# phhusson/SpeechSeparation

Measured on AMD Instinct MI355X. Metric: separated row-frames/sec, batch64 8s@16kHz, higher is better.
Workload: dtype f32 io/accumulate, fp16x2-split operands (22-bit operands, 3 f16 MFMA terms; a2*b2 term dropped)

## Files before the change

speechseparation_amd/csrc/api.hip:

```cpp
#include "api_internal.h"
#include "metrics_host.h"
#include "sections_host.h"

#include <cmath>
#include <cstdarg>
#include <cstdio>

namespace bsrnn::host {

std::atomic<long long> g_dbg[5];

static thread_local char g_err[512] = "";
int fail(int code, const char* fmt, ...)
{
    va_list ap;
    va_start(ap, fmt);
    vsnprintf(g_err, sizeof(g_err), fmt, ap);
    va_end(ap);
    return code;
}

hipError_t UploadRing::reserve(size_t bytes)
{
    if (bytes <= cap) return hipSuccess;
// ... 169 lines not shown
                (void)hipFree(t.d[0]);
                return fail(BSRNN_EHIP, "task table: %s", hipGetErrorString(e));
            }
        }
        c->chain_tasks.emplace(Ms[i], t);
    }
    return 0;
}
int ensure_tasks(bsrnn_ctx* c, int M) { return ensure_tasks(c, &M, 1); }

void gemm_slot(bsrnn_ctx* c, bool gemv, int slot, const float* X, int ldx, float* Y, int ldy, const float* R, int ldr,
               const float* Mul, int ldm, float* tap, int M, int epi, hipStream_t s)
{
    GemmLaunch g;
    memset(&g, 0, sizeof g);
    g.range_flag = c->d_range;
    g.jobs = c->d_jobs + c->slots.job0[slot];
    g.tiles = c->d_tiles + c->slots.tile0[slot];
    g.n_tiles = c->slots.ntiles[slot];
    g.tile_n = c->slots.tile_n[slot];
    g.X = X; g.ldx = ldx; g.Y = Y; g.ldy = ldy; g.R = R; g.ldr = ldr; g.Mul = Mul; g.ldm = ldm;
    g.tap = tap; g.ldt = c->LDP; g.M = M; g.epilogue = epi;
    if (gemv && M <= 2 * GEMV_MAX_FRAME_ROWS) launch_gemv(g, s);
    else launch_gemm(g, s);
}

static const PlanKnobs& plan_knobs()
{
    static const PlanKnobs knobs = [] {
        auto is = [](const char* name, const char* value) { const char* e = getenv(name); return e && !strcmp(e, value); };
        const char *tk = getenv("BSRNN_TIME_KERNEL"), *s8 = getenv("BSRNN_TIME_SEQ8");
        if (tk && *tk && strcmp(tk, "fused") && strcmp(tk, "v3")) fprintf(stderr, "bsrnn: unknown BSRNN_TIME_KERNEL='%s' (v3 | fused), using fused\n", tk);
        return PlanKnobs{!is("BSRNN_BAND_PAIR", "0"), !is("BSRNN_BAND_FC", "gemm"), !is("BSRNN_TIME_KERNEL", "v3"), s8 ? atoi(s8) : -1,
                         gemm_mode(), lstm_mode(), device_cus()};
    }();
    return knobs;
}
Flow plan_call(const bsrnn_ctx* c, int C, int T, bool gemv, bool overlap)
{
    return plan_call(c->K, C, T, gemv, overlap, plan_knobs(), PlanState{force_f32(), c->fused, c->band_pair_off, c->overlap_env, c->overlap_off});
}

struct Part {
    int C, T;
    Flow f;
    hipStream_t s;
    const float* Xf; float* Yf; float* tap;
    float *A1, *A2, *P, *Z0, *Z1, *HB0, *HB1, *H1;
    int* band_flags;
    const float* state_in; float* state_out;
    size_t state_slab;
    const float* wave; float* wave_out; int64_t n;
    const int64_t* lens;
    int64_t wave_stride, out_stride;
    const int2* tasks[2]; int n_tasks[2];
    const bsrnn_ctx::OvlTable* ovl;
    int ovl_base;
    hipEvent_t band_done[2];
    const int* row_frames;
};

Part make_part(bsrnn_ctx* c, int row0, int C, int T, hipStream_t s, int j = 0)
{
    Part p;
    memset(&p, 0, sizeof p);
    const size_t m0 = (size_t)row0 * T, KH = (size_t)c->K * HID;
    p.C = C; p.T = T; p.s = s;
// ... 37 lines not shown
    case MS_BANDSPLIT: {
        StageScope sc(c, ST_BANDSPLIT, s);
        if (f.chains) {
            ChainLaunch g;
            if (!chain_launch(c, p, CHAIN_SPLIT, g)) break;
            g.Xin = p.Xf; g.ldx = c->LDP; g.Z = p.Z0; g.ldz = KH;
            launch_mlp_chain(g, CHAIN_SPLIT, s);
            break;
        }
        gemm_slot(c, f.gemv, PRE0, p.Xf, c->LDP, p.A1, c->LDA, nullptr, 0, nullptr, 0, nullptr, M, EPI_LEAKY, s);
        gemm_slot(c, f.gemv, PRE2, p.A1, c->LDA, p.P, c->LDP, nullptr, 0, nullptr, 0, nullptr, M, EPI_LEAKY, s);
        gemm_slot(c, f.gemv, FC0, p.P, c->LDP, p.A1, c->LDA, nullptr, 0, nullptr, 0, nullptr, M, EPI_LEAKY, s);
        gemm_slot(c, f.gemv, FC2, p.A1, c->LDA, p.A2, c->LDA, nullptr, 0, nullptr, 0, nullptr, M, EPI_LEAKY, s);
        gemm_slot(c, f.gemv, FC4, p.A2, c->LDA, p.Z0, KH, nullptr, 0, nullptr, 0, nullptr, M, EPI_LINEAR, s);
        break;
    }
    case MS_BAND0: case MS_BAND1: {
        const int blk = stage == MS_BAND1;
        StageScope sc(c, ST_BAND_LSTM, s);
        if (f.band == BAND_SMALL) {
            launch_band_block_small(p.Z0, p.Z1, c->bandW16[blk][0], c->bandB[blk][0], c->bandW16[blk][1], c->bandB[blk][1],
                                    c->bandFc16[blk], c->bandFcB[blk], M, K, c->d_range, s);
            break;
        }
        const bool parts = f.band == BAND_PAIR_PARTS;
        const float* zi = parts && blk ? p.Z1 : p.Z0;
        if (f.band != BAND_LAYERS) {
            OvlConsumer oc = {nullptr, 0, 0, nullptr, 0, 2};
            const bool cons = p.ovl && blk;
            if (cons)
                oc = OvlConsumer{c->d_ovl + OVL_HEAD, p.T, c->overlap_sabotage ? 200000 : OVL_SPIN_LIMIT, p.ovl->band_order, p.ovl_base, f.seqs == 8 ? 3 : 2};
            launch_band_pair(zi, p.HB0, p.HB1, c->bandW16[blk][0], c->bandB[blk][0], c->bandW16[blk][1], c->bandB[blk][1], M, K, c->d_range, s,
                             parts ? c->bandFc16[blk] : nullptr, parts ? c->bandFcB[blk] : nullptr, p.band_flags, cons ? &oc : nullptr, nullptr, 0,
                             p.ovl ? p.band_done[blk] : nullptr);
            break;
        }
        launch_band_lstm(zi, p.HB0, c->bandW[blk][0], c->bandW16[blk][0], c->bandB[blk][0], M, K, 64, c->d_range, s, f.lstm_f32);
        launch_band_lstm(p.HB0, p.HB1, c->bandW[blk][1], c->bandW16[blk][1], c->bandB[blk][1], M, K, 128, c->d_range, s, f.lstm_f32);
        break;
    }
    case MS_BANDFC0: case MS_BANDFC1: {
        const int blk = stage == MS_BANDFC1;
        if (f.band == BAND_SMALL || f.band == BAND_PAIR_PARTS) break;
        StageScope sc(c, ST_BAND_FC, s);
        gemm_slot(c, f.gemv, BLK_FC0 + 2 * blk, p.HB1, 2 * HID, p.Z1, HID, p.Z0, HID, nullptr, 0, nullptr, M * K, EPI_RES, s);
        break;
    }
    case MS_TIME0: case MS_TIME1: {
        const int blk = stage == MS_TIME1;
        StageScope sc(c, ST_TIME_LSTM, s);
        const bool first_of_parts = f.band == BAND_PAIR_PARTS && !blk;
        OvlProducer op = {nullptr, nullptr, 0};
        if (p.ovl) op = OvlProducer{c->d_ovl + blk * c->ovl_stride, c->overlap_sabotage ? nullptr : c->d_ovl + blk * c->ovl_stride + OVL_HEAD, p.ovl_base};
        launch_time_lstm(first_of_parts ? p.Z0 : p.Z1, first_of_parts ? p.Z1 : (f.time_fc ? p.Z0 : p.H1), c->timeW[blk], c->timeW16[blk], c->timeB[blk],
                         p.state_in ? p.state_in + blk * p.state_slab : nullptr, p.state_out ? p.state_out + blk * p.state_slab : nullptr,
                         p.C, p.T, K, c->d_range, s, f.lstm_f32, f.seqs, f.time_fc ? c->timeFc16[blk] : nullptr, f.time_fc ? c->timeFcB[blk] : nullptr,
                         f.band == BAND_PAIR_PARTS ? p.HB1 : nullptr, p.ovl ? &op : nullptr, p.row_frames);
        break;
    }
    case MS_TIMEFC0: case MS_TIMEFC1: {
        const int blk = stage == MS_TIMEFC1;
        if (f.time_fc) break;
        StageScope sc(c, ST_TIME_FC, s);
        gemm_slot(c, f.gemv, BLK_FC1 + 2 * blk, p.H1, HID, p.Z0, HID, p.Z1, HID, nullptr, 0, nullptr, M * K, EPI_RES, s);
        break;
    }
    case MS_MASK: {
// ... 1754 lines not shown
```

speechseparation_amd/csrc/kernels.h:

```cpp
#pragma once
#include <hip/hip_runtime.h>
#include <stdint.h>

#include "descriptors.h"
#include "stream_rows_host.h"
#include "resample_bank_host.h"
#include "train_ragged_host.h"
#include "pool_host.h"
#include "convolve_host.h"
#include "convolve_stream_host.h"
#include "metrics_host.h"
#include "remix_host.h"
#include "critic_host.h"

namespace bsrnn {

enum GemmEpilogue {
    EPI_LINEAR = 0,
    EPI_LEAKY = 1,
    EPI_RES = 2,
    EPI_MASK = 3
};

struct GemmLaunch {
// ... 36 lines not shown
void launch_mlp_chain(const ChainLaunch& g, int chain, hipStream_t stream);

struct OvlProducer { int* resident; int* prog; int base; };
struct OvlConsumer { const int* prog; int T; int spin_limit; const int* order; int base; int wg_shift; };
constexpr int OVL_SPIN_LIMIT = 20000000;
void launch_ovl_gate(const int* resident, int target, int* range_flag, int spin_limit, hipStream_t stream);
int device_cus();
#if defined(__HIPCC__)
__device__ __forceinline__ bool ovl_wait_rows(const int* prog, int m_first, int m_last, int T, int K, int k_first, int k_last, int limit, int base, int wg_shift)
{
    typedef const int __attribute__((address_space(1)))* gci;
    const gci pg = (gci)prog;
    const int r_a = m_first / T, r_b = m_last / T;
    const unsigned long long t0 = __builtin_amdgcn_s_memrealtime();
    for (int r = r_a; r <= r_b; ++r) {
        const int t_last = r < r_b ? T - 1 : m_last - r * T;
        const int need = base + (t_last >> 2) + 1;
        for (int wg = (r * K + k_first) >> wg_shift; wg <= (r * K + k_last) >> wg_shift; ++wg)
            while (__hip_atomic_load(pg + wg, __ATOMIC_RELAXED, __HIP_MEMORY_SCOPE_AGENT) < need) {
                __builtin_amdgcn_s_sleep(16);
                if (__builtin_amdgcn_s_memrealtime() - t0 > (unsigned long long)limit) return false;
            }
    }
    __builtin_amdgcn_fence(__ATOMIC_ACQUIRE, "agent");
    asm volatile("s_waitcnt vmcnt(0)" ::: "memory");
    return true;
}
#endif

void launch_band_lstm(const float* xin, float* hout, const float* wpk, const void* wpk16, const float* bias,
                      int N, int L, int IN, int* range_flag, hipStream_t stream, bool f32);
void launch_band_pair(const float* z, float* hb0, float* hb1, const void* w0pk16, const float* bias0, const void* w1pk16, const float* bias1,
                      int N, int L, int* range_flag, hipStream_t stream, const void* fc16, const float* fcb, int* flags,
                      const OvlConsumer* ovl = nullptr, int* zero_words = nullptr, int zero_n = 0, hipEvent_t done = nullptr);
void launch_band_block_small(const float* zin, float* zout, const void* w0pk16, const float* bias0, const void* w1pk16, const float* bias1,
                             const void* fc16, const float* fcb, int N, int L, int* range_flag, hipStream_t stream);
int lstm_mode();
void launch_time_lstm(const float* zin, float* hout, const float* wpk, const void* wpk16, const float* bias,
                      const float* state_in, float* state_out, int R, int T, int K, int* range_flag, hipStream_t stream,
                      bool f32, int seqs, const void* fc16 = nullptr, const float* fcb = nullptr, const float* part = nullptr,
                      const OvlProducer* ovl = nullptr,
                      const int* row_frames = nullptr);

constexpr int LSTM_TRAIN_CHUNKS = 64;
constexpr int LSTM_TRAIN_MAX_CHUNKS = 256;
constexpr int GEMM_GROUP = 12;
struct TrainGemmJob {
    const float* A; const float* B; float* C; const float* bias;
    int lda, ldb, ldc;
    int M, N, K;
    int tiles_x, tiles_y, rpc;
};
struct TrainGemmGroup { TrainGemmJob j[GEMM_GROUP]; int first[GEMM_GROUP + 1]; int count; };
struct ReduceJob { const float* part; float* out1; float* out2; int n1, n2, chunks; };
struct ReduceGroup { ReduceJob j[GEMM_GROUP]; int first[GEMM_GROUP + 1]; int count; };
void launch_sgemm_group(TrainGemmGroup& g, int trans_b, int accumulate, int leaky, hipStream_t stream);
size_t tn_group_scratch_floats(const TrainGemmGroup& g);
void launch_sgemm_tn_group(const TrainGemmGroup& g, float* scratch, int L, int shift, hipStream_t stream);
size_t sgemm_tn_scratch_floats(int M, int N1, int N2);
void train_reduction_layout(int M, int N1, int N2, int out[2]);
size_t colsum_scratch_floats(int M, int cols);
void launch_sgemm(const float* A, int lda, const float* B, int ldb, int trans_b, float* C, int ldc, int M, int N, int K,
                  int accumulate, const float* bias, int leaky, hipStream_t stream);
void launch_sgemm_tn(const float* A, int lda, const float* B, int ldb, float* out, float* colsum, float* scratch, int M, int N1, int N2,
                     int L, int shift, hipStream_t stream);
void launch_colsum(const float* A, int lda, float* out, float* scratch, int M, int cols, hipStream_t stream);
void launch_adamw(float* p, const float* g, float* m, float* v, size_t n, float lr, double b1, double b2, float eps, float wd,
// ... 142 lines not shown
```

speechseparation_amd/csrc/lstm.hip:

```cpp
#include "kernels.h"
#include <hip/hip_ext.h>

#include <cstdio>
#include <cstdlib>
#include <cstring>
#include <type_traits>

namespace bsrnn {

typedef float v4f __attribute__((ext_vector_type(4)));

constexpr int BAND_NLDS = 2;
constexpr int BAND_NLDS64 = 0;

__device__ __forceinline__ float fast_sigmoid(float x)
{
    return __builtin_amdgcn_rcpf(1.0f + __expf(-x));
}
__device__ __forceinline__ float fast_tanh(float x)
{
    return 2.0f * __builtin_amdgcn_rcpf(1.0f + __expf(-2.0f * x)) - 1.0f;
}
__device__ __forceinline__ v4f exp2_4(const v4f x)
{
    return (v4f){__builtin_amdgcn_exp2f(x[0]), __builtin_amdgcn_exp2f(x[1]), __builtin_amdgcn_exp2f(x[2]), __builtin_amdgcn_exp2f(x[3])};
}
__device__ __forceinline__ v4f rcp4(const v4f x)
{
    return (v4f){__builtin_amdgcn_rcpf(x[0]), __builtin_amdgcn_rcpf(x[1]), __builtin_amdgcn_rcpf(x[2]), __builtin_amdgcn_rcpf(x[3])};
}

constexpr int BAND_OCC = 2;
template <int IN>
// ... 92 lines not shown
            c[r] = fg * c[r] + ig * gg;
            hbuf[nxt][(4 * q + r) * SH + 16 * wave + l15] = og * fast_tanh(c[r]);
        }
        if (more) xstore(nxt, xn);
        __syncthreads();
        if (n0 + o_row < N)
            *reinterpret_cast<float4*>(hout + ((size_t)(n0 + o_row) * L + t) * (2 * HID) + dir * HID + 4 * o_c4) =
                *reinterpret_cast<const float4*>(&hbuf[nxt][o_row * SH + 4 * o_c4]);
    }
}

typedef _Float16 h8v __attribute__((ext_vector_type(8)));
typedef _Float16 h4v __attribute__((ext_vector_type(4)));
typedef unsigned u4v __attribute__((ext_vector_type(4)));

__device__ __forceinline__ void split_h2(float v, _Float16& p0, _Float16& p1)
{
    asm("" : "+v"(v));
    p0 = (_Float16)v;
    p1 = (_Float16)__builtin_fmaf(-(float)p0, 2048.f, v * 2048.f);
}

template <int IN, bool PART>
struct BandLds {
    static constexpr int NLDS = IN == 128 ? BAND_NLDS : BAND_NLDS64;
    static constexpr int XPL = 0;
    static constexpr int HPL = XPL + 2 * 2 * IN * 16 * 2;
    static constexpr int W2 = HPL + 2 * 2 * HID * 16 * 2;
    static constexpr int BIAS = W2 + (NLDS ? 4 * NLDS * 4 * 64 : 1) * 16;
    static constexpr int FC = BIAS + (4 * HID + HID) * 4;
    static constexpr int BYTES = FC + (PART ? 4 * 2 * 2 * 64 : 1) * 16;
};

template <int IN, bool TRACE, bool PART>
__device__ __forceinline__ void band_layer_body(char* const lds, const int dir, const int tile,
                                                const float* __restrict__ xin, float* __restrict__ hout,
                                                const uint4* __restrict__ wpk, const float* __restrict__ bias,
                                                int N, int L, int* __restrict__ range_flag, unsigned long long* __restrict__ dbg,
                                                const uint4* __restrict__ wfc, const float* __restrict__ bfc)
{
    static_assert(!PART || IN == 2 * HID, "the fc share is formed by the second layer");
    unsigned long long tp[5] = {0, 0, 0, 0, 0}, tq = 0;
    auto stamp = [&](int k) { if (TRACE) { const unsigned long long now = __builtin_amdgcn_s_memrealtime(); tp[k] += now - tq; tq = now; } };
    if (TRACE) tq = __builtin_amdgcn_s_memrealtime();
    constexpr int NBX = IN / 32, NBH = HID / 32, NB = NBX + NBH;
    constexpr bool PLANES_IN = IN == 2 * HID;
    constexpr bool PLANES_OUT = IN == HID;
    constexpr int NLDS = IN == 128 ? BAND_NLDS : BAND_NLDS64;
    constexpr int XV = IN / 64;
    using LD = BandLds<IN, PART>;
    auto& xpl = *reinterpret_cast<_Float16 (*)[2][2][IN * 16]>(lds + LD::XPL);
    auto& hpl = *reinterpret_cast<_Float16 (*)[2][2][HID * 16]>(lds + LD::HPL);
    uint4* const w2lds = reinterpret_cast<uint4*>(lds + LD::W2);
    float* const bias_lds = reinterpret_cast<float*>(lds + LD::BIAS);
    uint4* const fclds = reinterpret_cast<uint4*>(lds + LD::FC);
    const int n0 = tile * 16;
    const int tid = threadIdx.x, lane = tid & 63, wave = tid >> 6;
    const int l15 = lane & 15, q = lane >> 4;

    h8v w[NB][4][2];
    {
        const uint4* wp = wpk + ((size_t)(dir * 4 + wave) * NB * 4 * 2) * 64 + lane;
#pragma unroll
        for (int b = 0; b < NB; ++b)
#pragma unroll
            for (int gte = 0; gte < 4; ++gte)
#pragma unroll
                for (int pc = 0; pc < 2; ++pc) {
                    const uint4 v = wp[((b * 4 + gte) * 2 + pc) * 64];
                    if (pc == 1 && b >= NB - NLDS)
                        w2lds[((wave * NLDS + (b - (NB - NLDS))) * 4 + gte) * 64 + lane] = v;
                    else
                        w[b][gte][pc] = __builtin_bit_cast(h8v, v);
                }
    }
    bias_lds[tid] = bias[dir * 256 + tid];
    if (PART) {
#pragma unroll
        for (int i = 0; i < 4; ++i) fclds[(wave * 4 + i) * 64 + lane] = wfc[((size_t)(wave * 4 + 2 * dir) * 2 + i) * 64 + lane];
    }
#pragma unroll
    for (int b = 0; b < NB; ++b)
#pragma unroll
        for (int gte = 0; gte < 4; ++gte) {
            asm volatile("" : "+v"(w[b][gte][0]));
            if (b < NB - NLDS) asm volatile("" : "+v"(w[b][gte][1]));
        }
    v4f cv = {0.f, 0.f, 0.f, 0.f};

    int xrow[XV], xcol[XV];
#pragma unroll
    for (int i = 0; i < XV; ++i) {
        const int u = tid + 256 * i;
        xrow[i] = u / (IN / 4);
        xcol[i] = u % (IN / 4);
    }
    auto xload = [&](int t, u4v* dst) {
#pragma unroll
        for (int i = 0; i < XV; ++i) {
            int row = n0 + xrow[i];
            row = row < N ? row : N - 1;
            dst[i] = *reinterpret_cast<const u4v*>(xin + ((size_t)row * L + t) * IN + 4 * xcol[i]);
        }
    };
    float amax = 0.f;
    auto xstore = [&](int slot, const u4v* src) {
#pragma unroll
        for (int i = 0; i < XV; ++i) {
            if (PLANES_IN) {
                const int piece = xcol[i] >> 4, k8 = xcol[i] & 15;
                *reinterpret_cast<u4v*>(&xpl[slot][piece][(k8 * 16 + xrow[i]) * 8]) = src[i];
            } else {
                const v4f v = __builtin_bit_cast(v4f, src[i]);
                h4v p0, p1;
#pragma unroll
                for (int e = 0; e < 4; ++e) {
                    amax = __builtin_fmaxf(amax, __builtin_fabsf(v[e]));
                    _Float16 a, b2;
                    split_h2(v[e], a, b2);
                    p0[e] = a; p1[e] = b2;
// ... 10 lines not shown
    const v4f zero4 = {0.f, 0.f, 0.f, 0.f};
    const int frag = (q * 16 + l15) * 8;
    const float* const bias_l = &bias_lds[16 * wave + 4 * q];
    auto block_mfma = [&](const int b, const h8v a0, const h8v a1) {
        h8v w2[4];
#pragma unroll
        for (int gte = 0; gte < 4; ++gte)
            w2[gte] = b >= NB - NLDS ? __builtin_bit_cast(h8v, w2lds[((wave * NLDS + (b - (NB - NLDS))) * 4 + gte) * 64 + lane]) : w[b][gte][1];
#pragma unroll
        for (int gte = 0; gte < 4; ++gte)
            hi[gte] = __builtin_amdgcn_mfma_f32_16x16x32_f16(w[b][gte][0], a0, b == 0 ? *reinterpret_cast<const v4f*>(bias_l + gte * HID) : hi[gte], 0, 0, 0);
#pragma unroll
        for (int gte = 0; gte < 4; ++gte) lo[gte] = __builtin_amdgcn_mfma_f32_16x16x32_f16(w[b][gte][0], a1, b == 0 ? zero4 : lo[gte], 0, 0, 0);
#pragma unroll
        for (int gte = 0; gte < 4; ++gte) lo[gte] = __builtin_amdgcn_mfma_f32_16x16x32_f16(w2[gte], a0, lo[gte], 0, 0, 0);
    };
    auto x_part = [&](int slot) {
        h8v a0 = *reinterpret_cast<const h8v*>(&xpl[slot][0][frag]);
        h8v a1 = *reinterpret_cast<const h8v*>(&xpl[slot][1][frag]);
#pragma unroll
        for (int b = 0; b < NBX; ++b) {
            h8v n0v = a0, n1v = a1;
            if (b + 1 < NBX) {
                n0v = *reinterpret_cast<const h8v*>(&xpl[slot][0][(b + 1) * 512 + frag]);
                n1v = *reinterpret_cast<const h8v*>(&xpl[slot][1][(b + 1) * 512 + frag]);
            }
            block_mfma(b, a0, a1);
            __builtin_amdgcn_sched_barrier(0);
            a0 = n0v; a1 = n1v;
        }
    };
    v4f fhi = zero4, flo = zero4;
    const float* const fb_l = bias_lds + 4 * HID + 16 * wave + 4 * q;
    if (PART && tid < HID) bias_lds[4 * HID + tid] = dir == 0 ? bfc[tid] : 0.f;
    auto fc_mfma = [&](const int b, const h8v a0, const h8v a1) {
        const h8v f1 = __builtin_bit_cast(h8v, fclds[(wave * 4 + 2 * b) * 64 + lane]);
        const h8v f2 = __builtin_bit_cast(h8v, fclds[(wave * 4 + 2 * b + 1) * 64 + lane]);
        fhi = __builtin_amdgcn_mfma_f32_16x16x32_f16(f1, a0, b == 0 ? *reinterpret_cast<const v4f*>(fb_l) : fhi, 0, 0, 0);
        flo = __builtin_amdgcn_mfma_f32_16x16x32_f16(f1, a1, b == 0 ? zero4 : flo, 0, 0, 0);
        flo = __builtin_amdgcn_mfma_f32_16x16x32_f16(f2, a0, flo, 0, 0, 0);
    };
    auto h_part = [&](int slot, const bool gates) {
        h8v a0 = *reinterpret_cast<const h8v*>(&hpl[slot][0][frag]);
        h8v a1 = *reinterpret_cast<const h8v*>(&hpl[slot][1][frag]);
#pragma unroll
        for (int b = 0; b < NBH; ++b) {
            h8v n0v = a0, n1v = a1;
            if (b + 1 < NBH) {
                n0v = *reinterpret_cast<const h8v*>(&hpl[slot][0][(b + 1) * 512 + frag]);
                n1v = *reinterpret_cast<const h8v*>(&hpl[slot][1][(b + 1) * 512 + frag]);
            }
            if (gates) block_mfma(NBX + b, a0, a1);
            __builtin_amdgcn_sched_barrier(0);
            if (PART) { fc_mfma(b, a0, a1); __builtin_amdgcn_sched_barrier(0); }
            a0 = n0v; a1 = n1v;
        }
    };

    {
        *reinterpret_cast<uint4*>(&hpl[1][0][0] + tid * 8) = make_uint4(0, 0, 0, 0);
        u4v x0[XV];
        xload(tmap(0), x0);
        xstore(0, x0);
        if (L > 1) { xload(tmap(1), x0); xstore(1, x0); }
    }
    u4v xn[XV];
    if (L > 2) xload(tmap(2), xn);
    __syncthreads();
    x_part(0);
    if (L > 2) __syncthreads();
    stamp(0);

    const int hoff = ((2 * wave + (q >> 1)) * 16 + l15) * 8 + 4 * (q & 1);
    const bool row_ok = n0 + l15 < N;
    const size_t grow = (size_t)(row_ok ? n0 + l15 : 0) * L;
    for (int step = 0; step < L; ++step) {
        const int t = tmap(step);
        const bool more2 = step + 2 < L;

        h_part((step + 1) & 1, true);
        if (PART && step > 0 && row_ok)
            *reinterpret_cast<v4f*>(hout + (grow + tmap(step - 1)) * (2 * HID) + dir * HID + 16 * wave + 4 * q) = fhi + flo * (1.f / 2048.f);
        stamp(1);

        {
            const v4f pi = hi[0] + lo[0] * (1.f / 2048.f), pf = hi[1] + lo[1] * (1.f / 2048.f);
            const v4f pg = hi[2] + lo[2] * (1.f / 2048.f), po = hi[3] + lo[3] * (1.f / 2048.f);
            const v4f ig = rcp4(1.0f + exp2_4(pi * -1.44269504f)), fg = rcp4(1.0f + exp2_4(pf * -1.44269504f));
            const v4f gg = 2.0f * rcp4(1.0f + exp2_4(pg * -2.88539008f)) - 1.0f, og = rcp4(1.0f + exp2_4(po * -1.44269504f));
            cv = fg * cv + ig * gg;
            const v4f hv4 = og * (2.0f * rcp4(1.0f + exp2_4(cv * -2.88539008f)) - 1.0f);
            if (more2) xstore(step & 1, xn);
            h4v p0, p1;
// ... 5 lines not shown
            }
            *reinterpret_cast<h4v*>(&hpl[step & 1][0][hoff]) = p0;
            *reinterpret_cast<h4v*>(&hpl[step & 1][1][hoff]) = p1;
            if (row_ok) {
                if (PLANES_OUT) {
                    _Float16* const hp = reinterpret_cast<_Float16*>(hout) + ((grow + t) * 2) * (2 * HID) + dir * HID + 16 * wave + 4 * q;
                    *reinterpret_cast<h4v*>(hp) = p0;
                    *reinterpret_cast<h4v*>(hp + 2 * HID) = p1;
                } else if (!PART) {
                    *reinterpret_cast<v4f*>(hout + (grow + t) * (2 * HID) + dir * HID + 16 * wave + 4 * q) = hv4;
                }
            }
        }
        if (step + 3 < L) xload(tmap(step + 3), xn);
        stamp(2);
        if (step + 1 < L) x_part((step + 1) & 1);
        stamp(3);
        __syncthreads();
        stamp(4);
    }
    if (PART) {
        h_part((L - 1) & 1, false);
        if (row_ok)
            *reinterpret_cast<v4f*>(hout + (grow + tmap(L - 1)) * (2 * HID) + dir * HID + 16 * wave + 4 * q) = fhi + flo * (1.f / 2048.f);
    }
    if (!(amax <= 65504.f) && range_flag) *range_flag = 1;
    if (TRACE && lane == 0 && blockIdx.x < 4 && blockIdx.y == 0) {
        unsigned long long* d = dbg + (blockIdx.x * 4 + wave) * 5;
#pragma unroll
        for (int k = 0; k < 5; ++k) d[k] = tp[k];
    }
}

__device__ __forceinline__ bool band_tile_of_block(int N, int& dir, int& tile, const int* __restrict__ order = nullptr)
{
    const int w = blockIdx.x & 15;
    dir = w >> 3;
    tile = (blockIdx.x >> 4) * 8 + (w & 7);
    if (order) tile = order[tile];
    return tile >= 0 && tile * 16 < N;
}

template <int IN, bool TRACE = false, bool PART = false>
__global__ __launch_bounds__(256, BAND_OCC) void band_lstm_h2_kernel(const float* __restrict__ xin, float* __restrict__ hout,
                                                              const uint4* __restrict__ wpk, const float* __restrict__ bias,
                                                              int N, int L, int* __restrict__ range_flag, unsigned long long* __restrict__ dbg,
                                                              const uint4* __restrict__ wfc = nullptr, const float* __restrict__ bfc = nullptr)
{
    __shared__ __attribute__((aligned(16))) char lds[BandLds<IN, PART>::BYTES];
    int dir, tile;
    if (!band_tile_of_block(N, dir, tile)) return;
    band_layer_body<IN, TRACE, PART>(lds, dir, tile, xin, hout, wpk, bias, N, L, range_flag, dbg, wfc, bfc);
}

template <bool PART>
__global__ __launch_bounds__(256, 2) void band_pair_h2_kernel(const float* __restrict__ z, float* hb0, float* __restrict__ hb1,
                                                              const uint4* __restrict__ w0, const float* __restrict__ b0,
                                                              const uint4* __restrict__ w1, const float* __restrict__ b1,
                                                              int N, int L, int* __restrict__ range_flag,
                                                              const uint4* __restrict__ wfc, const float* __restrict__ bfc,
                                                              int* flags, int sabotage, OvlConsumer ovl, int* zero_words, int zero_n)
{
    constexpr int B0 = BandLds<HID, false>::BYTES, B1 = BandLds<2 * HID, PART>::BYTES;
    __shared__ __attribute__((aligned(16))) char lds[B0 > B1 ? B0 : B1];
    __shared__ int partner_ok;
    if (zero_words && blockIdx.x == 0)
        for (int i = threadIdx.x; i < zero_n; i += 256) zero_words[i] = 0;
    int dir, tile;
    if (!band_tile_of_block(N, dir, tile, ovl.order)) return;
    if (ovl.prog) {
        if (threadIdx.x == 0) {
            const int m_last = tile * 16 + 15 < N ? tile * 16 + 15 : N - 1;
            partner_ok = ovl_wait_rows(ovl.prog, tile * 16, m_last, ovl.T, L, 0, L - 1, ovl.spin_limit, ovl.base, ovl.wg_shift) ? 1 : 0;
        }
        __syncthreads();
        if (!partner_ok) {
            if (threadIdx.x == 0 && range_flag) *range_flag = 5;
            return;
        }
        __syncthreads();
    }
    band_layer_body<HID, false, false>(lds, dir, tile, z, hb0, w0, b0, N, L, range_flag, nullptr, nullptr, nullptr);
    __builtin_amdgcn_s_waitcnt(0x0f70);
    __syncthreads();
    if (threadIdx.x == 0) {
        const int xcc = __builtin_amdgcn_s_getreg((3 << 11) | 20) & 15;
        const int epoch = ((__hip_atomic_load(&flags[2 * tile + dir], __ATOMIC_RELAXED, __HIP_MEMORY_SCOPE_AGENT) >> 4) + 1) & 0x7ffffff;
        __hip_atomic_store(&flags[2 * tile + dir], (epoch << 4) | (sabotage ? (xcc ^ 8) : xcc), __ATOMIC_RELAXED, __HIP_MEMORY_SCOPE_AGENT);
        int spins = 0, v;
        while (((v = __hip_atomic_load(&flags[2 * tile + (dir ^ 1)], __ATOMIC_RELAXED, __HIP_MEMORY_SCOPE_AGENT)) >> 4) != epoch) {
            __builtin_amdgcn_s_sleep(8);
            if (++spins > (1 << 22)) break;
        }
        partner_ok = (v >> 4) == epoch && (v & 15) == xcc;
    }
    __syncthreads();
    if (!partner_ok) {
        if (threadIdx.x == 0 && range_flag) *range_flag = 4;
        return;
    }
    __builtin_amdgcn_fence(__ATOMIC_ACQUIRE, "workgroup");
    asm volatile("buffer_inv sc0" ::: "memory");
    band_layer_body<2 * HID, false, PART>(lds, dir, tile, hb0, hb1, w1, b1, N, L, range_flag, nullptr, wfc, bfc);
}

void launch_band_pair(const float* z, float* hb0, float* hb1, const void* w0pk16, const float* bias0, const void* w1pk16, const float* bias1,
                      int N, int L, int* range_flag, hipStream_t stream, const void* fc16, const float* fcb, int* flags, const OvlConsumer* ovlp,
                      int* zero_words, int zero_n, hipEvent_t done)
{
    if (N <= 0 || L <= 0) return;
    OvlConsumer ovl = {nullptr, 0, 0, nullptr, 0, 2};
    if (ovlp) ovl = *ovlp;
    const dim3 grid((((N + 15) / 16 + 7) / 8) * 16), block(256);
    static const int sabotage = [] { const char* e = getenv("BSRNN_BAND_PAIR"); return (e && !strcmp(e, "mismatch")) ? 1 : 0; }();
    if (fc16)
        hipExtLaunchKernelGGL((band_pair_h2_kernel<true>), grid, block, 0, stream, nullptr, done, 0, z, hb0, hb1, (const uint4*)w0pk16, bias0, (const uint4*)w1pk16, bias1, N, L,
                              range_flag, (const uint4*)fc16, fcb, flags, sabotage, ovl, zero_words, zero_n);
    else
        hipExtLaunchKernelGGL((band_pair_h2_kernel<false>), grid, block, 0, stream, nullptr, done, 0, z, hb0, hb1, (const uint4*)w0pk16, bias0, (const uint4*)w1pk16, bias1, N, L,
                              range_flag, (const uint4*)nullptr, (const float*)nullptr, flags, sabotage, ovl, zero_words, zero_n);
}

void launch_band_lstm(const float* xin, float* hout, const float* wpk, const void* wpk16, const float* bias,
                      int N, int L, int IN, int* range_flag, hipStream_t stream, bool f32)
{
    if (N <= 0 || L <= 0) return;
    const dim3 block(256);
    if (!f32) {
        const dim3 grid((((N + 15) / 16 + 7) / 8) * 16);
        if (IN == 64)
            hipLaunchKernelGGL(band_lstm_h2_kernel<64>, grid, block, 0, stream, xin, hout, (const uint4*)wpk16, bias, N, L, range_flag, (unsigned long long*)nullptr);
        else
            hipLaunchKernelGGL(band_lstm_h2_kernel<128>, grid, block, 0, stream, xin, hout, (const uint4*)wpk16, bias, N, L, range_flag, (unsigned long long*)nullptr);
        return;
    }
    const dim3 grid((N + 15) / 16, 2);
    if (IN == 64)
        hipLaunchKernelGGL(band_lstm_kernel<64>, grid, block, 0, stream, xin, hout, wpk, bias, N, L);
    else
        hipLaunchKernelGGL(band_lstm_kernel<128>, grid, block, 0, stream, xin, hout, wpk, bias, N, L);
}

int lstm_mode()
{
    static const int mode = [] {
        const char* e = getenv("BSRNN_LSTM");
        if (!e || !*e || !strcmp(e, "fp16x2")) return (int)LSTM_FP16X2;
        if (!strcmp(e, "f32")) return (int)LSTM_F32;
        fprintf(stderr, "bsrnn: unknown BSRNN_LSTM='%s' (f32 | fp16x2), using fp16x2\n", e);
        return (int)LSTM_FP16X2;
    }();
    return mode;
}
// ... 1169 lines not shown
```

speechseparation_amd/csrc/plan_host.h:

```cpp
#pragma once
#include "descriptors.h"

#include <algorithm>
#include <cstddef>
#include <cstdint>
#include <utility>
#include <vector>

namespace bsrnn {

constexpr int MAX_PARTS = 4;
constexpr int OVL_HEAD = 16;

enum BandForm { BAND_SMALL, BAND_PAIR_PARTS, BAND_PAIR, BAND_LAYERS };
struct Flow {
    bool exact;
    bool lstm_f32;
    bool gemv;
    bool chains;
    int band;
    bool time_fc;
    int seqs, nwg;
    bool overlap;
};
struct PlanKnobs {
    bool band_pair, band_parts, time_fused;
    int seq8;
    int gemm_mode, lstm_mode;
    int cus;
};
struct PlanState { bool exact, fused, band_pair_off, overlap_env, overlap_off; };

inline Flow plan_call(int K, int C, int T, bool gemv, bool overlap, const PlanKnobs& kn, const PlanState& st)
{
    Flow f;
    const int M = C * T, N = C * K, cus = kn.cus;
    f.exact = st.exact;
    f.lstm_f32 = f.exact || kn.lstm_mode == LSTM_F32;
    const bool gemm16 = !f.exact && kn.gemm_mode != GEMM_F32;
    f.gemv = gemv && M <= GEMV_MAX_FRAME_ROWS;
    f.chains = st.fused && !f.exact && !f.gemv;
    f.time_fc = !f.lstm_f32 && gemm16 && kn.time_fused;
    const bool pair = !f.lstm_f32 && kn.band_pair && !st.band_pair_off;
    if (!f.lstm_f32 && gemm16 && M <= 8 && K <= BS_MAXL) f.band = BAND_SMALL;
    else if (pair && kn.band_parts && f.time_fc) f.band = BAND_PAIR_PARTS;
    else f.band = pair ? BAND_PAIR : BAND_LAYERS;
    f.seqs = f.time_fc && (kn.seq8 == 1 || (kn.seq8 < 0 && (N + 3) / 4 > cus)) ? 8 : 4;
    f.nwg = (N + f.seqs - 1) / f.seqs;
    f.overlap = overlap && st.overlap_env && !st.overlap_off && f.band == BAND_PAIR_PARTS && st.fused && f.nwg >= 32 && f.nwg <= cus - cus / 8 &&
                T >= 32 && T < (4 << OVL_EPOCH_SHIFT) - 8;
    return f;
}

inline size_t state_floats(int C, int K) { return (size_t)4 * 2 * C * K * HID; }
inline size_t state_slab_floats(int C, int K) { return (size_t)2 * 2 * C * K * HID; }

struct ChainTask { int desc, row0; };
inline void build_chain_tasks(const std::vector<ChainDesc>& ds, int M, std::vector<ChainTask>& out)
{
    out.clear();
    for (size_t di = 0; di < ds.size(); ++di)
        for (int r0 = 0; r0 < M; r0 += chain_rows(ds[di])) out.push_back(ChainTask{(int)di, r0});
}

inline int ovl_stride(int nwg) { return OVL_HEAD + ((nwg + 15) & ~15); }
struct OvlOrders { std::vector<int> band_order; std::vector<ChainTask> mask_tasks; };
inline OvlOrders ovl_orders(int M, int T, int nwg, int cus, const std::vector<ChainDesc>& ds )
{
    const int tiles = (M + 15) / 16, n_ord = ((tiles + 7) / 8) * 8;
    std::vector<int> order(tiles), ready(tiles);
    for (int t = 0; t < tiles; ++t) {
        const int m0 = 16 * t, m1 = std::min(M - 1, m0 + 15);
        order[t] = t;
        ready[t] = m0 / T != m1 / T ? T - 1 : m1 % T;
    }
    std::stable_sort(order.begin(), order.end(), [&](int a, int b) { return ready[a] < ready[b]; });
    order.resize(n_ord, -1);
    std::vector<ChainTask> tasks;
    build_chain_tasks(ds, M, tasks);
// ... 154 lines not shown
```

Measured before the change: 8.491 million.

## Run two band tiles per workgroup in band-pair kernel, reusing loaded weights

Splits the band LSTM layer body into a weight-load stage and a per-tile run stage, so a workgroup can process two 16-row tiles with one load of register and LDS weights. The planner picks two tiles per workgroup when tiles outnumber CUs, and an environment variable can force one or two. The second layer's weight loads are now issued before the cross-direction partner spin-wait and written to LDS afterwards, so the global-load latency overlaps the wait. In exchange the grid is halved, so there is less parallel slack. The partner handshake also now loops over both tiles' flags.

After: 8.800 million, median of 6. 1.04x the previous value.

```diff
diff --git a/speechseparation_amd/csrc/api.hip b/speechseparation_amd/csrc/api.hip
--- a/speechseparation_amd/csrc/api.hip
+++ b/speechseparation_amd/csrc/api.hip
@@ -225,7 +225,7 @@
         const char *tk = getenv("BSRNN_TIME_KERNEL"), *s8 = getenv("BSRNN_TIME_SEQ8");
         if (tk && *tk && strcmp(tk, "fused") && strcmp(tk, "v3")) fprintf(stderr, "bsrnn: unknown BSRNN_TIME_KERNEL='%s' (v3 | fused), using fused\n", tk);
         return PlanKnobs{!is("BSRNN_BAND_PAIR", "0"), !is("BSRNN_BAND_FC", "gemm"), !is("BSRNN_TIME_KERNEL", "v3"), s8 ? atoi(s8) : -1,
-                         gemm_mode(), lstm_mode(), device_cus()};
+                         gemm_mode(), lstm_mode(), device_cus(), is("BSRNN_BAND_PAIR", "tiles1") ? 1 : is("BSRNN_BAND_PAIR", "tiles2") ? 2 : 0};
     }();
     return knobs;
 }
@@ -329,7 +329,7 @@
                 oc = OvlConsumer{c->d_ovl + OVL_HEAD, p.T, c->overlap_sabotage ? 200000 : OVL_SPIN_LIMIT, p.ovl->band_order, p.ovl_base, f.seqs == 8 ? 3 : 2};
             launch_band_pair(zi, p.HB0, p.HB1, c->bandW16[blk][0], c->bandB[blk][0], c->bandW16[blk][1], c->bandB[blk][1], M, K, c->d_range, s,
                              parts ? c->bandFc16[blk] : nullptr, parts ? c->bandFcB[blk] : nullptr, p.band_flags, cons ? &oc : nullptr, nullptr, 0,
-                             p.ovl ? p.band_done[blk] : nullptr);
+                             p.ovl ? p.band_done[blk] : nullptr, f.band_tiles);
             break;
         }
         launch_band_lstm(zi, p.HB0, c->bandW[blk][0], c->bandW16[blk][0], c->bandB[blk][0], M, K, 64, c->d_range, s, f.lstm_f32);
diff --git a/speechseparation_amd/csrc/kernels.h b/speechseparation_amd/csrc/kernels.h
--- a/speechseparation_amd/csrc/kernels.h
+++ b/speechseparation_amd/csrc/kernels.h
@@ -92,7 +92,8 @@
                       int N, int L, int IN, int* range_flag, hipStream_t stream, bool f32);
 void launch_band_pair(const float* z, float* hb0, float* hb1, const void* w0pk16, const float* bias0, const void* w1pk16, const float* bias1,
                       int N, int L, int* range_flag, hipStream_t stream, const void* fc16, const float* fcb, int* flags,
-                      const OvlConsumer* ovl = nullptr, int* zero_words = nullptr, int zero_n = 0, hipEvent_t done = nullptr);
+                      const OvlConsumer* ovl = nullptr, int* zero_words = nullptr, int zero_n = 0, hipEvent_t done = nullptr,
+                      int tiles = 1);
 void launch_band_block_small(const float* zin, float* zout, const void* w0pk16, const float* bias0, const void* w1pk16, const float* bias1,
                              const void* fc16, const float* fcb, int N, int L, int* range_flag, hipStream_t stream);
 int lstm_mode();
diff --git a/speechseparation_amd/csrc/lstm.hip b/speechseparation_amd/csrc/lstm.hip
--- a/speechseparation_amd/csrc/lstm.hip
+++ b/speechseparation_amd/csrc/lstm.hip
@@ -1,4 +1,5 @@
 #include "kernels.h"
+#include "plan_host.h"
 #include <hip/hip_ext.h>
 
 #include <cstdio>
@@ -157,12 +158,81 @@
     static constexpr int BYTES = FC + (PART ? 4 * 2 * 2 * 64 : 1) * 16;
 };
 
+template <int IN, bool PART>
+struct BandW {
+    static constexpr int NB = IN / 32 + HID / 32;
+    static constexpr int NLDS = IN == 128 ? BAND_NLDS : BAND_NLDS64;
+    h8v w[NB][4][2];
+    uint4 w2[NLDS ? NLDS : 1][4];
+    uint4 fc[4];
+    float bias, bfc;
+};
+
+template <int IN, bool PART>
+__device__ __forceinline__ void band_issue_weights(BandW<IN, PART>& W, const int dir, const uint4* __restrict__ wpk, const float* __restrict__ bias,
+                                                   const uint4* __restrict__ wfc, const float* __restrict__ bfc)
+{
+    constexpr int NB = BandW<IN, PART>::NB, NLDS = BandW<IN, PART>::NLDS;
+    const int tid = threadIdx.x, lane = tid & 63, wave = tid >> 6;
+    const uint4* wp = wpk + ((size_t)(dir * 4 + wave) * NB * 4 * 2) * 64 + lane;
+#pragma unroll
+    for (int b = 0; b < NB; ++b)
+#pragma unroll
+        for (int gte = 0; gte < 4; ++gte)
+#pragma unroll
+            for (int pc = 0; pc < 2; ++pc) {
+                const uint4 v = wp[((b * 4 + gte) * 2 + pc) * 64];
+                if (pc == 1 && b >= NB - NLDS) W.w2[NLDS ? b - (NB - NLDS) : 0][gte] = v;
+                else W.w[b][gte][pc] = __builtin_bit_cast(h8v, v);
+            }
+    W.bias = bias[dir * 256 + tid];
+    if (PART) {
+#pragma unroll
+        for (int i = 0; i < 4; ++i) W.fc[i] = wfc[((size_t)(wave * 4 + 2 * dir) * 2 + i) * 64 + lane];
+        W.bfc = tid < HID && dir == 0 ? bfc[tid] : 0.f;
+    }
+}
+
+template <int IN, bool PART>
+__device__ __forceinline__ void band_commit_weights(BandW<IN, PART>& W, char* const lds)
+{
+    constexpr int NB = BandW<IN, PART>::NB, NLDS = BandW<IN, PART>::NLDS;
+    using LD = BandLds<IN, PART>;
+    uint4* const w2lds = reinterpret_cast<uint4*>(lds + LD::W2);
+    float* const bias_lds = reinterpret_cast<float*>(lds + LD::BIAS);
+    uint4* const fclds = reinterpret_cast<uint4*>(lds + LD::FC);
+    const int tid = threadIdx.x, lane = tid & 63, wave = tid >> 6;
+#pragma unroll
+    for (int b = 0; b < NLDS; ++b)
+#pragma unroll
+        for (int gte = 0; gte < 4; ++gte) w2lds[((wave * NLDS + b) * 4 + gte) * 64 + lane] = W.w2[b][gte];
+    bias_lds[tid] = W.bias;
+    if (PART) {
+#pragma unroll
+        for (int i = 0; i < 4; ++i) fclds[(wave * 4 + i) * 64 + lane] = W.fc[i];
+        if (tid < HID) bias_lds[4 * HID + tid] = W.bfc;
+    }
+#pragma unroll
+    for (int b = 0; b < NB; ++b)
+#pragma unroll
+        for (int gte = 0; gte < 4; ++gte) {
+            asm volatile("" : "+v"(W.w[b][gte][0]));
+            if (b < NB - NLDS) asm volatile("" : "+v"(W.w[b][gte][1]));
+        }
+}
+
+template <int IN, bool PART>
+__device__ __forceinline__ void band_load_weights(BandW<IN, PART>& W, char* const lds, const int dir, const uint4* __restrict__ wpk,
+                                                  const float* __restrict__ bias, const uint4* __restrict__ wfc, const float* __restrict__ bfc)
+{
+    band_issue_weights<IN, PART>(W, dir, wpk, bias, wfc, bfc);
+    band_commit_weights<IN, PART>(W, lds);
+}
+
 template <int IN, bool TRACE, bool PART>
-__device__ __forceinline__ void band_layer_body(char* const lds, const int dir, const int tile,
-                                                const float* __restrict__ xin, float* __restrict__ hout,
-                                                const uint4* __restrict__ wpk, const float* __restrict__ bias,
-                                                int N, int L, int* __restrict__ range_flag, unsigned long long* __restrict__ dbg,
-                                                const uint4* __restrict__ wfc, const float* __restrict__ bfc)
+__device__ __forceinline__ void band_run_tile(const BandW<IN, PART>& W, char* const lds, const int dir, const int tile,
+                                              const float* __restrict__ xin, float* __restrict__ hout,
+                                              int N, int L, int* __restrict__ range_flag, unsigned long long* __restrict__ dbg)
 {
     static_assert(!PART || IN == 2 * HID, "the fc share is formed by the second layer");
     unsigned long long tp[5] = {0, 0, 0, 0, 0}, tq = 0;
@@ -176,41 +246,15 @@
     using LD = BandLds<IN, PART>;
     auto& xpl = *reinterpret_cast<_Float16 (*)[2][2][IN * 16]>(lds + LD::XPL);
     auto& hpl = *reinterpret_cast<_Float16 (*)[2][2][HID * 16]>(lds + LD::HPL);
-    uint4* const w2lds = reinterpret_cast<uint4*>(lds + LD::W2);
-    float* const bias_lds = reinterpret_cast<float*>(lds + LD::BIAS);
-    uint4* const fclds = reinterpret_cast<uint4*>(lds + LD::FC);
+    const uint4* const w2lds = reinterpret_cast<const uint4*>(lds + LD::W2);
+    const float* const bias_lds = reinterpret_cast<const float*>(lds + LD::BIAS);
+    const uint4* const fclds = reinterpret_cast<const uint4*>(lds + LD::FC);
     const int n0 = tile * 16;
-    const int tid = threadIdx.x, lane = tid & 63, wave = tid >> 6;
+    int tid_ = threadIdx.x;
+    asm volatile("" : "+v"(tid_));
+    const int tid = tid_ & 255, lane = tid & 63, wave = tid >> 6;
     const int l15 = lane & 15, q = lane >> 4;
-
-    h8v w[NB][4][2];
-    {
-        const uint4* wp = wpk + ((size_t)(dir * 4 + wave) * NB * 4 * 2) * 64 + lane;
-#pragma unroll
-        for (int b = 0; b < NB; ++b)
-#pragma unroll
-            for (int gte = 0; gte < 4; ++gte)
-#pragma unroll
-                for (int pc = 0; pc < 2; ++pc) {
-                    const uint4 v = wp[((b * 4 + gte) * 2 + pc) * 64];
-                    if (pc == 1 && b >= NB - NLDS)
-                        w2lds[((wave * NLDS + (b - (NB - NLDS))) * 4 + gte) * 64 + lane] = v;
-                    else
-                        w[b][gte][pc] = __builtin_bit_cast(h8v, v);
-                }
-    }
-    bias_lds[tid] = bias[dir * 256 + tid];
-    if (PART) {
-#pragma unroll
-        for (int i = 0; i < 4; ++i) fclds[(wave * 4 + i) * 64 + lane] = wfc[((size_t)(wave * 4 + 2 * dir) * 2 + i) * 64 + lane];
-    }
-#pragma unroll
-    for (int b = 0; b < NB; ++b)
-#pragma unroll
-        for (int gte = 0; gte < 4; ++gte) {
-            asm volatile("" : "+v"(w[b][gte][0]));
-            if (b < NB - NLDS) asm volatile("" : "+v"(w[b][gte][1]));
-        }
+    const auto& w = W.w;
     v4f cv = {0.f, 0.f, 0.f, 0.f};
 
     int xrow[XV], xcol[XV];
@@ -287,7 +331,6 @@
     };
     v4f fhi = zero4, flo = zero4;
     const float* const fb_l = bias_lds + 4 * HID + 16 * wave + 4 * q;
-    if (PART && tid < HID) bias_lds[4 * HID + tid] = dir == 0 ? bfc[tid] : 0.f;
     auto fc_mfma = [&](const int b, const h8v a0, const h8v a1) {
         const h8v f1 = __builtin_bit_cast(h8v, fclds[(wave * 4 + 2 * b) * 64 + lane]);
         const h8v f2 = __builtin_bit_cast(h8v, fclds[(wave * 4 + 2 * b + 1) * 64 + lane]);
@@ -313,7 +356,9 @@
     };
 
     {
-        *reinterpret_cast<uint4*>(&hpl[1][0][0] + tid * 8) = make_uint4(0, 0, 0, 0);
+        unsigned zw;
+        asm volatile("v_mov_b32 %0, 0" : "=v"(zw));
+        *reinterpret_cast<uint4*>(&hpl[1][0][0] + tid * 8) = make_uint4(zw, zw, zw, zw);
         u4v x0[XV];
         xload(tmap(0), x0);
         xstore(0, x0);
@@ -385,13 +430,30 @@
     }
 }
 
-__device__ __forceinline__ bool band_tile_of_block(int N, int& dir, int& tile, const int* __restrict__ order = nullptr)
+template <int TILES>
+__device__ __forceinline__ int band_tiles_of_block(int N, int& dir, int (&tile)[TILES], const int* __restrict__ order)
 {
     const int w = blockIdx.x & 15;
     dir = w >> 3;
-    tile = (blockIdx.x >> 4) * 8 + (w & 7);
-    if (order) tile = order[tile];
-    return tile >= 0 && tile * 16 < N;
+    const int slot = (blockIdx.x >> 4) * 8 + (w & 7);
+    const int n_tiles = (N + 15) / 16, n_ord = (n_tiles + 7) & ~7;
+    int nt = 0;
+#pragma unroll
+    for (int i = 0; i < TILES; ++i) {
+        const int e = slot * TILES + i;
+        int t = e;
+        if (order) t = e < n_ord ? order[e] : -1;
+        tile[i] = t;
+        if (nt == i && t >= 0 && t < n_tiles) nt = i + 1;
+    }
+    return nt;
+}
+__device__ __forceinline__ bool band_tile_of_block(int N, int& dir, int& tile)
+{
+    int t[1];
+    const int nt = band_tiles_of_block<1>(N, dir, t, nullptr);
+    tile = t[0];
+    return nt != 0;
 }
 
 template <int IN, bool TRACE = false, bool PART = false>
@@ -403,10 +465,12 @@
     __shared__ __attribute__((aligned(16))) char lds[BandLds<IN, PART>::BYTES];
     int dir, tile;
     if (!band_tile_of_block(N, dir, tile)) return;
-    band_layer_body<IN, TRACE, PART>(lds, dir, tile, xin, hout, wpk, bias, N, L, range_flag, dbg, wfc, bfc);
-}
-
-template <bool PART>
+    BandW<IN, PART> W;
+    band_load_weights<IN, PART>(W, lds, dir, wpk, bias, wfc, bfc);
+    band_run_tile<IN, TRACE, PART>(W, lds, dir, tile, xin, hout, N, L, range_flag, dbg);
+}
+
+template <bool PART, int TILES>
 __global__ __launch_bounds__(256, 2) void band_pair_h2_kernel(const float* __restrict__ z, float* hb0, float* __restrict__ hb1,
                                                               const uint4* __restrict__ w0, const float* __restrict__ b0,
                                                               const uint4* __restrict__ w1, const float* __restrict__ b1,
@@ -414,38 +478,66 @@
                                                               const uint4* __restrict__ wfc, const float* __restrict__ bfc,
                                                               int* flags, int sabotage, OvlConsumer ovl, int* zero_words, int zero_n)
 {
+    static_assert(TILES == 1 || TILES == 2, "one or two tiles per workgroup");
     constexpr int B0 = BandLds<HID, false>::BYTES, B1 = BandLds<2 * HID, PART>::BYTES;
     __shared__ __attribute__((aligned(16))) char lds[B0 > B1 ? B0 : B1];
     __shared__ int partner_ok;
     if (zero_words && blockIdx.x == 0)
         for (int i = threadIdx.x; i < zero_n; i += 256) zero_words[i] = 0;
-    int dir, tile;
-    if (!band_tile_of_block(N, dir, tile, ovl.order)) return;
-    if (ovl.prog) {
-        if (threadIdx.x == 0) {
-            const int m_last = tile * 16 + 15 < N ? tile * 16 + 15 : N - 1;
-            partner_ok = ovl_wait_rows(ovl.prog, tile * 16, m_last, ovl.T, L, 0, L - 1, ovl.spin_limit, ovl.base, ovl.wg_shift) ? 1 : 0;
-        }
-        __syncthreads();
-        if (!partner_ok) {
-            if (threadIdx.x == 0 && range_flag) *range_flag = 5;
-            return;
-        }
-        __syncthreads();
-    }
-    band_layer_body<HID, false, false>(lds, dir, tile, z, hb0, w0, b0, N, L, range_flag, nullptr, nullptr, nullptr);
+    int dir, tl[TILES];
+    const int nt = band_tiles_of_block<TILES>(N, dir, tl, ovl.order);
+    if (!nt) return;
+    auto tile_of = [&](int i) { return TILES == 2 && i ? tl[TILES - 1] : tl[0]; };
+    {
+        BandW<HID, false> W;
+        band_load_weights<HID, false>(W, lds, dir, w0, b0, nullptr, nullptr);
+        for (int i = 0; i < nt; ++i) {
+            const int tile = tile_of(i);
+            if (i) __syncthreads();
+            if (ovl.prog) {
+                if (threadIdx.x == 0) {
+                    const int m_last = tile * 16 + 15 < N ? tile * 16 + 15 : N - 1;
+                    partner_ok = ovl_wait_rows(ovl.prog, tile * 16, m_last, ovl.T, L, 0, L - 1, ovl.spin_limit, ovl.base, ovl.wg_shift) ? 1 : 0;
+                }
+                __syncthreads();
+                if (!partner_ok) {
+                    if (threadIdx.x == 0 && range_flag) *range_flag = 5;
+                    return;
+                }
+                __syncthreads();
+            }
+            band_run_tile<HID, false, false>(W, lds, dir, tile, z, hb0, N, L, range_flag, nullptr);
+        }
+    }
     __builtin_amdgcn_s_waitcnt(0x0f70);
     __syncthreads();
+    int epoch[TILES], xcc = 0;
     if (threadIdx.x == 0) {
-        const int xcc = __builtin_amdgcn_s_getreg((3 << 11) | 20) & 15;
-        const int epoch = ((__hip_atomic_load(&flags[2 * tile + dir], __ATOMIC_RELAXED, __HIP_MEMORY_SCOPE_AGENT) >> 4) + 1) & 0x7ffffff;
-        __hip_atomic_store(&flags[2 * tile + dir], (epoch << 4) | (sabotage ? (xcc ^ 8) : xcc), __ATOMIC_RELAXED, __HIP_MEMORY_SCOPE_AGENT);
-        int spins = 0, v;
-        while (((v = __hip_atomic_load(&flags[2 * tile + (dir ^ 1)], __ATOMIC_RELAXED, __HIP_MEMORY_SCOPE_AGENT)) >> 4) != epoch) {
-            __builtin_amdgcn_s_sleep(8);
-            if (++spins > (1 << 22)) break;
-        }
-        partner_ok = (v >> 4) == epoch && (v & 15) == xcc;
+        xcc = __builtin_amdgcn_s_getreg((3 << 11) | 20) & 15;
+#pragma unroll
+        for (int i = 0; i < TILES; ++i) {
+            if (i >= nt) break;
+            int* const mine = &flags[2 * tl[i] + dir];
+            epoch[i] = ((__hip_atomic_load(mine, __ATOMIC_RELAXED, __HIP_MEMORY_SCOPE_AGENT) >> 4) + 1) & 0x7ffffff;
+            __hip_atomic_store(mine, (epoch[i] << 4) | (sabotage ? (xcc ^ 8) : xcc), __ATOMIC_RELAXED, __HIP_MEMORY_SCOPE_AGENT);
+        }
+    }
+    BandW<2 * HID, PART> W;
+    band_issue_weights<2 * HID, PART>(W, dir, w1, b1, wfc, bfc);
+    if (threadIdx.x == 0) {
+        int ok = 1;
+#pragma unroll
+        for (int i = 0; i < TILES; ++i) {
+            if (i >= nt) break;
+            const int* const theirs = &flags[2 * tl[i] + (dir ^ 1)];
+            int spins = 0, v;
+            while (((v = __hip_atomic_load(theirs, __ATOMIC_RELAXED, __HIP_MEMORY_SCOPE_AGENT)) >> 4) != epoch[i]) {
+                __builtin_amdgcn_s_sleep(8);
+                if (++spins > (1 << 22)) break;
+            }
+            ok &= (v >> 4) == epoch[i] && (v & 15) == xcc;
+        }
+        partner_ok = ok;
     }
     __syncthreads();
     if (!partner_ok) {
@@ -454,24 +546,28 @@
     }
     __builtin_amdgcn_fence(__ATOMIC_ACQUIRE, "workgroup");
     asm volatile("buffer_inv sc0" ::: "memory");
-    band_layer_body<2 * HID, false, PART>(lds, dir, tile, hb0, hb1, w1, b1, N, L, range_flag, nullptr, wfc, bfc);
+    band_commit_weights<2 * HID, PART>(W, lds);
+    for (int i = 0; i < nt; ++i) {
+        if (i) __syncthreads();
+        band_run_tile<2 * HID, false, PART>(W, lds, dir, tile_of(i), hb0, hb1, N, L, range_flag, nullptr);
+    }
 }
 
 void launch_band_pair(const float* z, float* hb0, float* hb1, const void* w0pk16, const float* bias0, const void* w1pk16, const float* bias1,
                       int N, int L, int* range_flag, hipStream_t stream, const void* fc16, const float* fcb, int* flags, const OvlConsumer* ovlp,
-                      int* zero_words, int zero_n, hipEvent_t done)
+                      int* zero_words, int zero_n, hipEvent_t done, int tiles)
 {
     if (N <= 0 || L <= 0) return;
     OvlConsumer ovl = {nullptr, 0, 0, nullptr, 0, 2};
     if (ovlp) ovl = *ovlp;
-    const dim3 grid((((N + 15) / 16 + 7) / 8) * 16), block(256);
+    const dim3 grid(band_pair_grid(N, tiles)), block(256);
     static const int sabotage = [] { const char* e = getenv("BSRNN_BAND_PAIR"); return (e && !strcmp(e, "mismatch")) ? 1 : 0; }();
-    if (fc16)
-        hipExtLaunchKernelGGL((band_pair_h2_kernel<true>), grid, block, 0, stream, nullptr, done, 0, z, hb0, hb1, (const uint4*)w0pk16, bias0, (const uint4*)w1pk16, bias1, N, L,
-                              range_flag, (const uint4*)fc16, fcb, flags, sabotage, ovl, zero_words, zero_n);
-    else
-        hipExtLaunchKernelGGL((band_pair_h2_kernel<false>), grid, block, 0, stream, nullptr, done, 0, z, hb0, hb1, (const uint4*)w0pk16, bias0, (const uint4*)w1pk16, bias1, N, L,
-                              range_flag, (const uint4*)nullptr, (const float*)nullptr, flags, sabotage, ovl, zero_words, zero_n);
+    auto go = [&](auto kernel, const void* fc, const float* fb) {
+        hipExtLaunchKernelGGL(kernel, grid, block, 0, stream, nullptr, done, 0, z, hb0, hb1, (const uint4*)w0pk16, bias0, (const uint4*)w1pk16, bias1, N, L,
+                              range_flag, (const uint4*)fc, fb, flags, sabotage, ovl, zero_words, zero_n);
+    };
+    if (fc16) { if (tiles == 2) go(band_pair_h2_kernel<true, 2>, fc16, fcb); else go(band_pair_h2_kernel<true, 1>, fc16, fcb); }
+    else { if (tiles == 2) go(band_pair_h2_kernel<false, 2>, nullptr, nullptr); else go(band_pair_h2_kernel<false, 1>, nullptr, nullptr); }
 }
 
 void launch_band_lstm(const float* xin, float* hout, const float* wpk, const void* wpk16, const float* bias,
diff --git a/speechseparation_amd/csrc/plan_host.h b/speechseparation_amd/csrc/plan_host.h
--- a/speechseparation_amd/csrc/plan_host.h
+++ b/speechseparation_amd/csrc/plan_host.h
@@ -22,14 +22,24 @@
     bool time_fc;
     int seqs, nwg;
     bool overlap;
+    int band_tiles;
 };
 struct PlanKnobs {
     bool band_pair, band_parts, time_fused;
     int seq8;
     int gemm_mode, lstm_mode;
     int cus;
+    int band_tiles = 0;
 };
 struct PlanState { bool exact, fused, band_pair_off, overlap_env, overlap_off; };
+
+inline int band_pair_tiles(int N, int cus, int force = 0)
+{
+    if (force == 1 || force == 2) return force;
+    return 2 * ((N + 15) / 16) > 2 * cus ? 2 : 1;
+}
+inline int band_pair_slots(int N, int tiles) { const int nt = (N + 15) / 16; return tiles == 2 ? (nt + 1) / 2 : nt; }
+inline int band_pair_grid(int N, int tiles) { return (band_pair_slots(N, tiles) + 7) / 8 * 16; }
 
 inline Flow plan_call(int K, int C, int T, bool gemv, bool overlap, const PlanKnobs& kn, const PlanState& st)
 {
@@ -45,6 +55,7 @@
     if (!f.lstm_f32 && gemm16 && M <= 8 && K <= BS_MAXL) f.band = BAND_SMALL;
     else if (pair && kn.band_parts && f.time_fc) f.band = BAND_PAIR_PARTS;
     else f.band = pair ? BAND_PAIR : BAND_LAYERS;
+    f.band_tiles = band_pair_tiles(M, cus, kn.band_tiles);
     f.seqs = f.time_fc && (kn.seq8 == 1 || (kn.seq8 < 0 && (N + 3) / 4 > cus)) ? 8 : 4;
     f.nwg = (N + f.seqs - 1) / f.seqs;
     f.overlap = overlap && st.overlap_env && !st.overlap_off && f.band == BAND_PAIR_PARTS && st.fused && f.nwg >= 32 && f.nwg <= cus - cus / 8 &&
```
